# simonamtoft/downsampled-diffusion

Measured on AMD Instinct MI355X. Metric: images/sec (T=1000 sampling), 256x256 dDDPM-x3, higher is better.
Workload: dtype f32

## Files before the change

downsampled-diffusion_amd/csrc/level_chain.h:

```cpp
#pragma once
#include "ddk_internal.h"

namespace ddk {

constexpr int CH_MAX_OPS = 24;
enum ChainKind {
    CH_CONV3 = 0,
    CH_CONV1 = 1,
    CH_ATTN = 2,
    CH_UPT = 3
};
enum ChainFlag {
    CHF_WAIT = 1,
    CHF_SIGNAL = 2,
    CHF_ADD_KEEP = 4,
    CHF_SAVE_KEEP = 8,
    CHF_ADD_KEEP2 = 16,
    CHF_SAVE_KEEP2 = 32,
    CHF_KEEP_FROM_SRC = 64,
    CHF_NO_OUT = 128,
    CHF_NO_GN = 256,
    CHF_DOWN = 512
};

struct ChainOp {
    const float* src0;
    const float* src1;
    const float* w;
    const float* bias;
    const float* gamma;
    const float* beta;
    float* out;
    int c0, c1, kind, flags, temb_off, n_out;
};

struct ChainParams {
    ChainOp op[CH_MAX_OPS];
    const float* temb;
    const long long* temb_rows;
    unsigned* cnt;
    unsigned* done;
    unsigned* fail;
    int n_ops, B, temb_stride;
    float gn_eps, ln_eps;
    int hw;
};

bool level_chain_device_ok();
size_t level_chain_lds_bytes();
int level_chain_launch(const ChainParams& p, hipStream_t st);
int level_chain_init_device();

}
```

downsampled-diffusion_amd/csrc/level_chain.hip:

```cpp
#include "level_chain.h"
#include "cluster_sync.h"
#include "conv_common.h"

#include <atomic>
#include <cstdlib>
#include <type_traits>
#include <utility>

namespace ddk {

typedef float f32x4 __attribute__((ext_vector_type(4)));

constexpr int LC_BIG = 18432;
constexpr int LC_PP = 36;
constexpr int LC_QP = 100;
constexpr int LC_RED = LC_BIG;
constexpr int LC_TILE = LC_RED + 64;
constexpr int LC_KS = LC_TILE + 576;
constexpr int LC_VS = LC_KS + 512;
constexpr int LC_QS = LC_VS + 512;
constexpr int LC_CS = LC_QS + 528;
constexpr int LC_SMAX = LC_CS + 1152;
constexpr int LC_ROWSTAT = LC_SMAX + 32;
constexpr int LC_CFOLD = LC_ROWSTAT + 32;
constexpr int LC_MISC = LC_CFOLD + 192;
constexpr int LC_PF = LC_MISC + 4;
constexpr int LC_FLOATS = LC_PF + 256;

size_t level_chain_lds_bytes() { return 100 * 1024; }
static_assert(LC_FLOATS * 4 <= 100 * 1024, "LDS carve-up");

__device__ __forceinline__ void ld_sc1_x1(f32x4& a, const float* pa) {
    asm volatile("global_load_dwordx4 %0, %1, off sc1\n\ts_waitcnt vmcnt(0)" : "=&v"(a) : "v"(pa) : "memory");
}
__device__ __forceinline__ void ld_sc1_x2(f32x4& a, f32x4& b, const float* pa, const float* pb) {
    asm volatile("global_load_dwordx4 %0, %2, off sc1\n\tglobal_load_dwordx4 %1, %3, off sc1\n\ts_waitcnt vmcnt(0)"
                 : "=&v"(a), "=&v"(b) : "v"(pa), "v"(pb) : "memory");
}
__device__ __forceinline__ void ld_sc1_x4(f32x4& a, f32x4& b, f32x4& c, f32x4& d, const float* pa, const float* pb, const float* pc, const float* pd) {
    asm volatile("global_load_dwordx4 %0, %4, off sc1\n\tglobal_load_dwordx4 %1, %5, off sc1\n\tglobal_load_dwordx4 %2, %6, off sc1\n\t"
                 "global_load_dwordx4 %3, %7, off sc1\n\ts_waitcnt vmcnt(0)"
                 : "=&v"(a), "=&v"(b), "=&v"(c), "=&v"(d) : "v"(pa), "v"(pb), "v"(pc), "v"(pd) : "memory");
}
__device__ __forceinline__ void st_sc1(float* p, f32x4 v) { asm volatile("global_store_dwordx4 %0, %1, off sc1\n\ts_nop 1" :: "v"(p), "v"(v) : "memory"); }

#ifdef DDK_TUNING
__device__ unsigned long long g_lc_stamps[9 * CH_MAX_OPS * 8];
#define LC_STAMP(c, k, i)                                                                                                   \
    do {                                                                                                                    \
        if ((c).tid == 0 && (c).watch >= 0) g_lc_stamps[((c).watch * CH_MAX_OPS + (k)) * 8 + (i)] = __builtin_amdgcn_s_memrealtime(); \
    } while (0)
#else
#define LC_STAMP(c, k, i) do { } while (0)
// ... 10 lines not shown
    const int b = __builtin_bit_cast(int, v);
    const float r0 = __builtin_bit_cast(float, __builtin_amdgcn_readlane(b, 0)), r1 = __builtin_bit_cast(float, __builtin_amdgcn_readlane(b, 16));
    const float r2 = __builtin_bit_cast(float, __builtin_amdgcn_readlane(b, 32)), r3 = __builtin_bit_cast(float, __builtin_amdgcn_readlane(b, 48));
    return (r0 + r1) + (r2 + r3);
}

template <int... I, class F>
__device__ __forceinline__ void static_for_lc_impl(std::integer_sequence<int, I...>, F&& f) { (f(std::integral_constant<int, I>{}), ...); }
template <int N, class F>
__device__ __forceinline__ void static_for_lc(F&& f) { static_for_lc_impl(std::make_integer_sequence<int, N>{}, f); }

struct ChainCtx {
    float* lds;
    int tid, lane, wave, b, nt;
    unsigned signals;
    float keep, keep2;
    float* misc;
    unsigned pf_dst;
    int nwaves, units3;
    int slot, slots;
    int watch, k;
};

__device__ __forceinline__ void chain_wait(const ChainParams& p, ChainCtx& c) {
    int* dead = reinterpret_cast<int*>(c.misc);
    if (c.tid == 0 && !*dead && cl_wait_ge<1>(p.cnt + c.b * 32, 8u * c.signals, p.fail)) *dead = 1;
    __syncthreads();
}

__device__ __forceinline__ void chain_prefetch(const ChainOp& o, const ChainCtx& c) {
    const int cin = o.c0 + o.c1;
    const float* base;
    int lines;
    if (o.kind == CH_ATTN) {
        if (c.nt >= 4) return;
        base = o.w + (size_t)c.nt * (cin >> 5) * 3072;
        lines = (cin >> 5) * 3072 / 32;
    } else {
        const int taps = o.kind == CH_CONV3 ? c.units3 : o.kind == CH_UPT ? 16 : 1;
        base = o.w + (size_t)c.nt * taps * (cin >> 5) * 1024;
        lines = taps * (cin >> 5) * 1024 / 32;
    }
    const int share = (lines + c.slots - 1) / c.slots;
    const int first = c.slot * share;
    const int n = lines - first < share ? lines - first : share;
    for (int i = c.wave * 64; i < n; i += c.nwaves * 64) {
        int line = first + i + c.lane;
        line = line < first + n ? line : first + n - 1;
        lds_dma16(base + (size_t)line * 32, c.pf_dst);
    }
}

__device__ __forceinline__ void chain_finish(const ChainParams& p, const ChainOp& o, ChainCtx& c, float y, int n0) {
    if (o.flags & CHF_ADD_KEEP) y += c.keep;
    if (o.flags & CHF_ADD_KEEP2) y += c.keep2;
    if (o.flags & CHF_SAVE_KEEP) c.keep = y;
    if (o.flags & CHF_SAVE_KEEP2) c.keep2 = y;
    if (!(o.flags & CHF_NO_OUT)) {
        const int yb = __builtin_bit_cast(int, y);
        const float y0 = __builtin_bit_cast(float, __builtin_amdgcn_update_dpp(0, yb, 0x00, 0xF, 0xF, true));
        const float y1 = __builtin_bit_cast(float, __builtin_amdgcn_update_dpp(0, yb, 0x55, 0xF, 0xF, true));
        const float y2 = __builtin_bit_cast(float, __builtin_amdgcn_update_dpp(0, yb, 0xAA, 0xF, 0xF, true));
        const float y3 = __builtin_bit_cast(float, __builtin_amdgcn_update_dpp(0, yb, 0xFF, 0xF, 0xF, true));
        if ((c.lane & 3) == 0) {
            float* dst = o.out + ((long long)c.b * 16 + (c.tid >> 5)) * o.n_out + n0 + (c.tid & 31);
            const f32x4 v{y0, y1, y2, y3};
            if (o.flags & CHF_SIGNAL) st_sc1(dst, v);
            else *reinterpret_cast<f32x4*>(dst) = v;
        }
    }
    if (o.flags & CHF_SIGNAL) {
        asm volatile("s_waitcnt vmcnt(0)" ::: "memory");
        if (c.lane == 0) {
            unsigned* lcnt = reinterpret_cast<unsigned*>(c.misc) + 1;
            if ((atomicAdd(lcnt, 1u) & 7u) == 7u) __hip_atomic_fetch_add(p.cnt + c.b * 32, 1u, __ATOMIC_RELAXED, __HIP_MEMORY_SCOPE_AGENT);
        }
    }
}

__device__ __forceinline__ void chain_stage(const ChainOp& o, ChainCtx& c, int cin, int pitch) {
    const int q4 = cin >> 2;
    auto addr = [&](int idx) -> const float* {
        const int row = idx / q4, ch = (idx - row * q4) << 2;
        const long long r = (long long)c.b * 16 + row;
        return ch < o.c0 ? o.src0 + r * o.c0 + ch : o.src1 + r * o.c1 + (ch - o.c0);
    };
    auto put = [&](int idx, f32x4 v) {
        const int row = idx / q4, ch = (idx - row * q4) << 2;
        *reinterpret_cast<f32x4*>(c.lds + row * pitch + ch) = v;
    };
    if (cin == 512) {
        f32x4 v0, v1, v2, v3;
        ld_sc1_x4(v0, v1, v2, v3, addr(c.tid), addr(c.tid + 512), addr(c.tid + 1024), addr(c.tid + 1536));
        put(c.tid, v0); put(c.tid + 512, v1); put(c.tid + 1024, v2); put(c.tid + 1536, v3);
    } else if (cin == 256) {
        f32x4 v0, v1;
        ld_sc1_x2(v0, v1, addr(c.tid), addr(c.tid + 512));
        put(c.tid, v0); put(c.tid + 512, v1);
    } else {
        f32x4 v0;
        ld_sc1_x1(v0, addr(c.tid));
        put(c.tid, v0);
    }
    if (c.tid < q4) *reinterpret_cast<f32x4*>(c.lds + 16 * pitch + (c.tid << 2)) = f32x4{0.f, 0.f, 0.f, 0.f};
}

__device__ __forceinline__ void chain_stage64(const ChainOp& o, ChainCtx& c) {
    const float* src = o.src0 + (long long)c.b * 64 * 256;
#pragma unroll
    for (int r0 = 0; r0 < 4096; r0 += 2048) {
        f32x4 v0, v1, v2, v3;
        ld_sc1_x4(v0, v1, v2, v3, src + (size_t)(r0 + c.tid) * 4, src + (size_t)(r0 + c.tid + 512) * 4, src + (size_t)(r0 + c.tid + 1024) * 4,
                  src + (size_t)(r0 + c.tid + 1536) * 4);
        auto put = [&](int idx, f32x4 v) { *reinterpret_cast<f32x4*>(c.lds + (idx >> 6) * 260 + ((idx & 63) << 2)) = v; };
        put(r0 + c.tid, v0); put(r0 + c.tid + 512, v1); put(r0 + c.tid + 1024, v2); put(r0 + c.tid + 1536, v3);
    }
    if (c.tid < 64) *reinterpret_cast<f32x4*>(c.lds + 64 * 260 + (c.tid << 2)) = f32x4{0.f, 0.f, 0.f, 0.f};
}

template <int NU>
__device__ __forceinline__ void chain_conv(const ChainParams& p, const ChainOp& o, ChainCtx& c) {
    float* lds = c.lds;
    const int tid = c.tid, lane = c.lane, wave = c.wave;
    const int m = lane & 15, kq = lane >> 4;
    const int n0 = c.nt << 5;
    const int cin = o.c0 + o.c1, pitch = cin + 4, nch = cin >> 5;
    const int taps = o.kind == CH_CONV3 ? 9 : 1;

    const float* wl = o.w + (size_t)c.nt * taps * nch * 1024 + lane * 4;
    float4 bA[2][2], bB[2][2], bC[2][2];
    int ltap = 0, lchunk = wave;
    auto norm = [&](int& tap, int& chunk) {
        while (chunk >= nch) { chunk -= nch; ++tap; }
    };
    norm(ltap, lchunk);
    auto load_b = [&](float4 (&bq)[2][2]) {
        const int unit = ltap < taps ? ltap * nch + lchunk : taps * nch - 1;
        const float* wp = wl + (size_t)unit * 1024;
        bq[0][0] = *reinterpret_cast<const float4*>(wp);
        bq[0][1] = *reinterpret_cast<const float4*>(wp + 256);
        bq[1][0] = *reinterpret_cast<const float4*>(wp + 512);
        bq[1][1] = *reinterpret_cast<const float4*>(wp + 768);
        lchunk += 8;
        norm(ltap, lchunk);
    };
    load_b(bA);
    load_b(bB);
    load_b(bC);
    const int col = tid & 31, row = tid >> 5;
    const int ch = n0 + col;
    float ga = 1.f, be = 0.f, sh = 0.f;
    if (o.kind == CH_CONV3 && !(o.flags & CHF_NO_GN)) { ga = o.gamma[ch]; be = o.beta[ch]; }
    if (o.temb_off >= 0) {
        const long long tr = p.temb_rows ? p.temb_rows[c.b] : c.b;
        sh = p.temb[tr * p.temb_stride + o.temb_off + ch];
    }
    const float cb = o.bias ? o.bias[ch] : 0.f;
    if (o.flags & CHF_KEEP_FROM_SRC) c.keep = o.src0[((long long)c.b * 16 + row) * o.c0 + ch];
    if (c.k + 1 < p.n_ops) chain_prefetch(p.op[c.k + 1], c);
    const bool down = NU == 1 && (o.flags & CHF_DOWN);

    LC_STAMP(c, c.k, 0);
    if (o.flags & CHF_WAIT) chain_wait(p, c);
    else __syncthreads();
    LC_STAMP(c, c.k, 1);
    if (down) chain_stage64(o, c);
    else chain_stage(o, c, cin, pitch);
    __syncthreads();
    LC_STAMP(c, c.k, 2);

    f32x4 acc[2];
    acc[0] = acc[1] = f32x4{0.f, 0.f, 0.f, 0.f};
    const int py = m >> 2, px = m & 3;
    if constexpr (NU > 0) {
        int a_tap[9];
#pragma unroll
        for (int t = 0; t < 9; ++t) {
            if (down) {
                const int yy = 2 * py + t / 3 - 1, xx = 2 * px + t % 3 - 1;
                const bool ok = (unsigned)yy < 8u && (unsigned)xx < 8u;
                a_tap[t] = (ok ? yy * 8 + xx : 64) * pitch + kq * 8 + (wave << 5);
            } else {
                const int yy = py + t / 3 - 1, xx = px + t % 3 - 1;
                const bool ok = (unsigned)yy < 4u && (unsigned)xx < 4u;
                a_tap[t] = (ok ? yy * 4 + xx : 16) * pitch + kq * 8 + (wave << 5);
            }
        }
        auto compute_at = [&](int t, int sub, const float4 (&bq)[2][2]) {
            const float* ap = lds + a_tap[t] + sub * 256;
            const float4 a0 = *reinterpret_cast<const float4*>(ap), a1 = *reinterpret_cast<const float4*>(ap + 4);
            const float av[8] = {a0.x, a0.y, a0.z, a0.w, a1.x, a1.y, a1.z, a1.w};
#pragma unroll
// ... 24 lines not shown
            const float* ap = lds + srow * pitch + (cchunk << 5) + kq * 8;
            const float4 a0 = *reinterpret_cast<const float4*>(ap), a1 = *reinterpret_cast<const float4*>(ap + 4);
            const float av[8] = {a0.x, a0.y, a0.z, a0.w, a1.x, a1.y, a1.z, a1.w};
#pragma unroll
            for (int kk = 0; kk < 8; ++kk) {
                acc[0] = __builtin_amdgcn_mfma_f32_16x16x4f32(av[kk], reinterpret_cast<const float*>(&bq[0][0])[kk], acc[0], 0, 0, 0);
                acc[1] = __builtin_amdgcn_mfma_f32_16x16x4f32(av[kk], reinterpret_cast<const float*>(&bq[1][0])[kk], acc[1], 0, 0, 0);
            }
            cchunk += 8;
            norm(ctap, cchunk);
        };
        while (ctap < taps) {
            compute(bA);
            load_b(bA);
            if (ctap < taps) compute(bB);
            load_b(bB);
            if (ctap < taps) compute(bC);
            load_b(bC);
        }
    }

    LC_STAMP(c, c.k, 3);
    __syncthreads();
#pragma unroll
    for (int nb = 0; nb < 2; ++nb)
#pragma unroll
        for (int r = 0; r < 4; ++r) lds[(wave * 16 + kq * 4 + r) * LC_PP + nb * 16 + m] = acc[nb][r];
    __syncthreads();
    float v = lds[row * LC_PP + col];
#pragma unroll
    for (int w = 1; w < 8; ++w) v += lds[(w * 16 + row) * LC_PP + col];
    v += cb;
    float y = v;
    if (o.kind == CH_CONV3 && !(o.flags & CHF_NO_GN)) {
        float* red = lds + LC_RED;
        const float mw = wave_sum_dpp(v) * (1.0f / 64.0f);
        const float dw = v - mw;
        const float m2w = wave_sum_dpp(dw * dw);
        if (lane == 0) { red[2 * wave] = mw; red[2 * wave + 1] = m2w; }
        __syncthreads();
        float msum = red[0], m2 = red[1];
#pragma unroll
        for (int w = 1; w < 8; ++w) { msum += red[2 * w]; m2 += red[2 * w + 1]; }
        const float mean = msum * 0.125f;
        float dev = 0.f;
#pragma unroll
        for (int w = 0; w < 8; ++w) { const float dm = red[2 * w] - mean; dev += dm * dm; }
        const float var = (m2 + 64.0f * dev) * (1.0f / 512.0f);
        const float rstd = 1.0f / sqrtf(var + p.gn_eps);
        y = mish_f((v - mean) * rstd * ga + be) + sh;
    }
    chain_finish(p, o, c, y, n0);
    if (o.flags & CHF_SIGNAL) ++c.signals;
    LC_STAMP(c, c.k, 4);
// ... 2 lines not shown
__device__ __forceinline__ void chain_upt(const ChainParams& p, const ChainOp& o, ChainCtx& c) {
    float* lds = c.lds;
    const int tid = c.tid, lane = c.lane, wave = c.wave;
    const int m = lane & 15, kq = lane >> 4;
    const int n0 = c.nt << 5;
    const int cin = o.c0, pitch = cin + 4, nch = cin >> 5;
    const float* wl = o.w + ((size_t)c.nt * 16 * nch + wave) * 1024 + lane * 4;
    float4 bA[2][2], bB[2][2], bC[2][2];
    int lu = 0;
    auto load_b = [&](float4 (&bq)[2][2]) {
        const float* wp = wl + (size_t)(lu < 16 ? lu : 15) * nch * 1024;
        bq[0][0] = *reinterpret_cast<const float4*>(wp);
        bq[0][1] = *reinterpret_cast<const float4*>(wp + 256);
        bq[1][0] = *reinterpret_cast<const float4*>(wp + 512);
        bq[1][1] = *reinterpret_cast<const float4*>(wp + 768);
        ++lu;
    };
    load_b(bA);
    load_b(bB);
    load_b(bC);
    const int col = tid & 31, row = tid >> 5;
    const float cb = o.bias ? o.bias[n0 + col] : 0.f;
    if (c.k + 1 < p.n_ops) chain_prefetch(p.op[c.k + 1], c);
    LC_STAMP(c, c.k, 0);
    if (o.flags & CHF_WAIT) chain_wait(p, c);
    else __syncthreads();
    LC_STAMP(c, c.k, 1);
    chain_stage(o, c, cin, pitch);
    __syncthreads();
    LC_STAMP(c, c.k, 2);
    f32x4 acc[4][2];
#pragma unroll
    for (int ph = 0; ph < 4; ++ph) acc[ph][0] = acc[ph][1] = f32x4{0.f, 0.f, 0.f, 0.f};
    const int y = m >> 2, x = m & 3;
    auto unit = [&](auto phc, auto tpc, const float4 (&bq)[2][2]) {
        constexpr int ph = decltype(phc)::value, tp = decltype(tpc)::value;
        constexpr int pyy = ph >> 1, pxx = ph & 1, ty = tp >> 1, tx = tp & 1;
        constexpr int dy = pyy == 0 ? (ty == 0 ? 0 : -1) : (ty == 0 ? 1 : 0);
        constexpr int dx = pxx == 0 ? (tx == 0 ? 0 : -1) : (tx == 0 ? 1 : 0);
        const int yy = y + dy, xx = x + dx;
        const bool ok = (unsigned)yy < 4u && (unsigned)xx < 4u;
        const float* ap = lds + (ok ? yy * 4 + xx : 16) * pitch + (wave << 5) + kq * 8;
        const float4 a0 = *reinterpret_cast<const float4*>(ap), a1 = *reinterpret_cast<const float4*>(ap + 4);
        const float av[8] = {a0.x, a0.y, a0.z, a0.w, a1.x, a1.y, a1.z, a1.w};
#pragma unroll
        for (int kk = 0; kk < 8; ++kk) {
            acc[ph][0] = __builtin_amdgcn_mfma_f32_16x16x4f32(av[kk], reinterpret_cast<const float*>(&bq[0][0])[kk], acc[ph][0], 0, 0, 0);
            acc[ph][1] = __builtin_amdgcn_mfma_f32_16x16x4f32(av[kk], reinterpret_cast<const float*>(&bq[1][0])[kk], acc[ph][1], 0, 0, 0);
        }
    };
    static_for_lc<16>([&](auto uc) {
        constexpr int u = decltype(uc)::value;
        using PH = std::integral_constant<int, u / 4>;
        using TP = std::integral_constant<int, u % 4>;
        if constexpr (u % 3 == 0) { unit(PH{}, TP{}, bA); load_b(bA); }
        else if constexpr (u % 3 == 1) { unit(PH{}, TP{}, bB); load_b(bB); }
        else { unit(PH{}, TP{}, bC); load_b(bC); }
    });
    LC_STAMP(c, c.k, 3);
    __syncthreads();
#pragma unroll
    for (int ph = 0; ph < 4; ++ph)
#pragma unroll
        for (int nb = 0; nb < 2; ++nb)
#pragma unroll
            for (int r = 0; r < 4; ++r) lds[((wave * 4 + ph) * 16 + kq * 4 + r) * LC_PP + nb * 16 + m] = acc[ph][nb][r];
    __syncthreads();
    float yv[4];
#pragma unroll
    for (int ph = 0; ph < 4; ++ph) {
        float s = lds[(ph * 16 + row) * LC_PP + col];
#pragma unroll
        for (int w = 1; w < 8; ++w) s += lds[((w * 4 + ph) * 16 + row) * LC_PP + col];
        yv[ph] = s + cb;
    }
    {
        float g[4][4];
#pragma unroll
        for (int k = 0; k < 4; ++k) {
            const int yb = __builtin_bit_cast(int, yv[k]);
            g[k][0] = __builtin_bit_cast(float, __builtin_amdgcn_update_dpp(0, yb, 0x00, 0xF, 0xF, true));
            g[k][1] = __builtin_bit_cast(float, __builtin_amdgcn_update_dpp(0, yb, 0x55, 0xF, 0xF, true));
            g[k][2] = __builtin_bit_cast(float, __builtin_amdgcn_update_dpp(0, yb, 0xAA, 0xF, 0xF, true));
            g[k][3] = __builtin_bit_cast(float, __builtin_amdgcn_update_dpp(0, yb, 0xFF, 0xF, 0xF, true));
        }
        const int j = lane & 3;
        f32x4 v;
#pragma unroll
        for (int q = 0; q < 4; ++q) v[q] = j == 0 ? g[0][q] : j == 1 ? g[1][q] : j == 2 ? g[2][q] : g[3][q];
        const int oy = 2 * (row >> 2) + (j >> 1), ox = 2 * (row & 3) + (j & 1);
        float* dst = o.out + ((long long)c.b * 64 + oy * 8 + ox) * o.n_out + n0 + (col & ~3);
        if (o.flags & CHF_SIGNAL) st_sc1(dst, v);
        else *reinterpret_cast<f32x4*>(dst) = v;
    }
    if (o.flags & CHF_SIGNAL) {
        asm volatile("s_waitcnt vmcnt(0)" ::: "memory");
        if (lane == 0) {
            unsigned* lcnt = reinterpret_cast<unsigned*>(c.misc) + 1;
            if ((atomicAdd(lcnt, 1u) & 7u) == 7u) __hip_atomic_fetch_add(p.cnt + c.b * 32, 1u, __ATOMIC_RELAXED, __HIP_MEMORY_SCOPE_AGENT);
        }
        ++c.signals;
    }
    LC_STAMP(c, c.k, 4);
}

__device__ __forceinline__ void chain_attn(const ChainParams& p, const ChainOp& o, ChainCtx& c) {
    float* lds = c.lds;
    const int tid = c.tid, lane = c.lane, wave = c.wave;
    if (c.k + 1 < p.n_ops) chain_prefetch(p.op[c.k + 1], c);
    if (c.k + 2 < p.n_ops) chain_prefetch(p.op[c.k + 2], c);
    if (c.nt < 4) {
        const int h = c.nt;
        const int m = lane & 15, kq = lane >> 4;
        const int C = o.c0, pitch = C + 4, nch = C >> 5;
        float* xs = lds;
        float* ks = lds + LC_KS;
        float* vs = lds + LC_VS;
        float* qs = lds + LC_QS;
        float* cs = lds + LC_CS;
        float* smax = lds + LC_SMAX;
        float* rowstat = lds + LC_ROWSTAT;
        float* cfold = lds + LC_CFOLD;
        const float* wl = o.w + (size_t)h * nch * 3072 + lane * 4;
        float4 bq[6][2];
        {
            const int chunk = wave < nch ? wave : nch - 1;
            const float* wp = wl + (size_t)chunk * 3072;
#pragma unroll
            for (int nb = 0; nb < 6; ++nb) {
                bq[nb][0] = *reinterpret_cast<const float4*>(wp + nb * 512);
                bq[nb][1] = *reinterpret_cast<const float4*>(wp + nb * 512 + 256);
            }
        }
        if (tid < 192) {
            const int n = tid % 96;
            const int colw = (n >> 5) * 128 + h * 32 + (n & 31);
            cfold[tid] = tid < 96 ? o.gamma[colw] : o.beta[colw];
        }
        LC_STAMP(c, c.k, 0);
        if (o.flags & CHF_WAIT) chain_wait(p, c);
        else __syncthreads();
        LC_STAMP(c, c.k, 1);
        chain_stage(o, c, C, pitch);
        __syncthreads();
        LC_STAMP(c, c.k, 2);
        {
            const int row = tid >> 5, sub = tid & 31;
            float s1 = 0.f;
            for (int ch = sub * 4; ch < C; ch += 128) {
                const float4 v = *reinterpret_cast<const float4*>(xs + row * pitch + ch);
                s1 += (v.x + v.y) + (v.z + v.w);
            }
#pragma unroll
            for (int of = 1; of < 32; of <<= 1) s1 += __shfl_xor(s1, of, 64);
            const float inv_c = 1.0f / (float)C;
            const float mean = s1 * inv_c;
            float s2 = 0.f;
            for (int ch = sub * 4; ch < C; ch += 128) {
                const float4 v = *reinterpret_cast<const float4*>(xs + row * pitch + ch);
                const float a0 = v.x - mean, a1 = v.y - mean, a2 = v.z - mean, a3 = v.w - mean;
                s2 += (a0 * a0 + a1 * a1) + (a2 * a2 + a3 * a3);
            }
#pragma unroll
            for (int of = 1; of < 32; of <<= 1) s2 += __shfl_xor(s2, of, 64);
            if (sub == 0) {
                const float r = 1.0f / (sqrtf(s2 * inv_c) + p.ln_eps);
                rowstat[2 * row] = r;
                rowstat[2 * row + 1] = r * mean;
// ... 2 lines not shown
        f32x4 acc[6];
#pragma unroll
        for (int nb = 0; nb < 6; ++nb) acc[nb] = f32x4{0.f, 0.f, 0.f, 0.f};
        for (int chunk = wave; chunk < nch; chunk += 8) {
            const float* ap = xs + m * pitch + (chunk << 5) + kq * 8;
            const float4 a0 = *reinterpret_cast<const float4*>(ap), a1 = *reinterpret_cast<const float4*>(ap + 4);
            const float av[8] = {a0.x, a0.y, a0.z, a0.w, a1.x, a1.y, a1.z, a1.w};
#pragma unroll
            for (int kk = 0; kk < 8; ++kk)
#pragma unroll
                for (int nb = 0; nb < 6; ++nb)
                    acc[nb] = __builtin_amdgcn_mfma_f32_16x16x4f32(av[kk], reinterpret_cast<const float*>(&bq[nb][0])[kk], acc[nb], 0, 0, 0);
            if (chunk + 8 < nch) {
                const float* wp = wl + (size_t)(chunk + 8) * 3072;
#pragma unroll
                for (int nb = 0; nb < 6; ++nb) {
                    bq[nb][0] = *reinterpret_cast<const float4*>(wp + nb * 512);
                    bq[nb][1] = *reinterpret_cast<const float4*>(wp + nb * 512 + 256);
                }
            }
        }
        LC_STAMP(c, c.k, 3);
        __syncthreads();
#pragma unroll
        for (int nb = 0; nb < 6; ++nb)
#pragma unroll
            for (int r = 0; r < 4; ++r) xs[(wave * 16 + kq * 4 + r) * LC_QP + nb * 16 + m] = acc[nb][r];
        __syncthreads();
        for (int e = tid; e < 16 * 96; e += 512) {
            const int row = e / 96, n = e - row * 96;
            float s = xs[row * LC_QP + n];
#pragma unroll
            for (int w = 1; w < 8; ++w) s += xs[(w * 16 + row) * LC_QP + n];
            const float v = rowstat[2 * row] * s - rowstat[2 * row + 1] * cfold[n] + cfold[96 + n];
            const int sel = n >> 5, d = n & 31;
            if (sel == 0) qs[row * 33 + d] = v;
            else if (sel == 1) ks[row * 32 + d] = v;
            else vs[row * 32 + d] = v;
        }
        __syncthreads();
        if (tid < 32) {
            float mx = ks[tid];
#pragma unroll
            for (int n = 1; n < 16; ++n) mx = fmaxf(mx, ks[n * 32 + tid]);
            smax[tid] = mx;
        }
        __syncthreads();
        ks[tid] = __expf(ks[tid] - smax[tid & 31]);
        __syncthreads();
        {
            const int d = tid >> 4, e0 = (tid & 15) << 1;
            float a0 = 0.f, a1 = 0.f, den = 0.f;
#pragma unroll
            for (int n = 0; n < 16; ++n) {
                const float kd = ks[n * 32 + d];
                a0 += kd * vs[n * 32 + e0];
                a1 += kd * vs[n * 32 + e0 + 1];
                den += kd;
            }
            const float inv = 1.0f / den;
            cs[d * 36 + e0] = a0 * inv;
            cs[d * 36 + e0 + 1] = a1 * inv;
        }
        __syncthreads();
        const int n = tid >> 5, e = tid & 31;
        float y = 0.f;
#pragma unroll
        for (int d = 0; d < 32; ++d) y += qs[n * 33 + d] * cs[d * 36 + e];
        chain_finish(p, o, c, y, h * 32);
    } else {
        if (o.flags & CHF_WAIT) chain_wait(p, c);
        if ((o.flags & CHF_SIGNAL) && tid == 0) __hip_atomic_fetch_add(p.cnt + c.b * 32, 1u, __ATOMIC_RELAXED, __HIP_MEMORY_SCOPE_AGENT);
    }
    if (o.flags & CHF_SIGNAL) ++c.signals;
    LC_STAMP(c, c.k, 4);
}

__global__ __launch_bounds__(512) void level_chain_kernel(const ChainParams p) {
    extern __shared__ __align__(16) float lds[];
    ChainCtx c;
    c.lds = lds;
    c.tid = threadIdx.x;
    c.lane = c.tid & 63;
    c.wave = __builtin_amdgcn_readfirstlane(c.tid >> 6);
    c.nt = blockIdx.x & 7;
    c.misc = lds + LC_MISC;
    c.pf_dst = (unsigned)(size_t)(__attribute__((address_space(3))) float*)(lds + LC_PF);
    c.nwaves = 8;
    c.units3 = 9;
    c.watch = blockIdx.x == 0 ? 0 : blockIdx.x == 100 ? 1 : blockIdx.x == 255 ? 2 : -1;
    c.k = 0;
    if (c.tid == 0) { *reinterpret_cast<int*>(lds + LC_MISC) = 0; reinterpret_cast<unsigned*>(lds + LC_MISC)[1] = 0u; }
    __syncthreads();
    const int slots = gridDim.x >> 3;
    c.slot = blockIdx.x >> 3;
    c.slots = slots;
    for (int b = blockIdx.x >> 3; b < p.B; b += slots) {
        c.b = b;
        c.signals = 0;
        c.keep = c.keep2 = 0.f;
        chain_prefetch(p.op[0], c);
        for (int k = 0; k < p.n_ops; ++k) {
            const ChainOp& o = p.op[k];
            c.k = k;
            if (o.kind == CH_ATTN) chain_attn(p, o, c);
            else if (o.kind == CH_UPT) chain_upt(p, o, c);
            else if (o.kind == CH_CONV1) chain_conv<0>(p, o, c);
            else if (o.c0 + o.c1 == 256) chain_conv<1>(p, o, c);
            else if (o.c0 + o.c1 == 512) chain_conv<2>(p, o, c);
            else chain_conv<0>(p, o, c);
        }
        __syncthreads();
        if (c.tid == 0) cl_depart(p.cnt + b * 32, p.done + b * 32, 8u);
    }
}

constexpr int L8_P = 260;
constexpr int L8_IMG = 65 * L8_P;
constexpr int L8_VP = 36;
constexpr int L8_VBUF = 16 * 16 * L8_VP;
constexpr int L8_V = L8_IMG;
constexpr int L8_KS = L8_V;
constexpr int L8_VS = L8_KS + 2048;
constexpr int L8_QS = L8_VS + 2048;
constexpr int L8_CS = L8_QS + 2112;
constexpr int L8_RED = L8_V + 2 * L8_VBUF;
constexpr int L8_SMAX = L8_RED + 64;
constexpr int L8_ROWSTAT = L8_SMAX + 320;
constexpr int L8_CFOLD = L8_ROWSTAT + 128;
constexpr int L8_MISC = L8_CFOLD + 192;
constexpr int L8_PF = L8_MISC + 4;
constexpr int L8_FLOATS = L8_PF + 256;
static_assert(L8_CS + 1152 <= L8_RED, "attention arrays fit the V buffers");
static_assert(L8_FLOATS * 4 <= 160 * 1024, "LDS carve-up (8x8)");
static_assert(2 * 64 * LC_QP <= L8_IMG && 8 * 64 * LC_PP <= 2 * L8_VBUF, "partial tiles fit");

// ... 82 lines not shown
        }
    };
    const int tt = (tid >> 5) & 15, col = tid & 31, ch = n0 + col;
    const int tty = tt >> 2, ttx = tt & 3;
    float ga = 1.f, be = 0.f, sh = 0.f, cb = 0.f;
    if (matrix) {
        load_b(0, bA);
        load_b(1, bB);
        ga = o.gamma[ch]; be = o.beta[ch];
        if (o.temb_off >= 0) {
            const long long tr = p.temb_rows ? p.temb_rows[c.b] : c.b;
            sh = p.temb[tr * p.temb_stride + o.temb_off + ch];
        }
        if (o.bias) cb = o.bias[ch];
        if (o.flags & CHF_KEEP_FROM_SRC) {
#pragma unroll
            for (int k = 0; k < 4; ++k)
                kp.keep[k] = o.src0[((long long)c.b * 64 + (2 * tty + (k >> 1)) * 8 + 2 * ttx + (k & 1)) * o.c0 + ch];
        }
    }
    if (c.k + 1 < p.n_ops) chain_prefetch(p.op[c.k + 1], c);

    LC_STAMP(c, c.k, 0);
    if (o.flags & CHF_WAIT) chain_wait(p, c);
    else __syncthreads();
    LC_STAMP(c, c.k, 1);

    f32x4 acc[2][2];
    acc[0][0] = acc[0][1] = acc[1][0] = acc[1][1] = f32x4{0.f, 0.f, 0.f, 0.f};
    if (!matrix) {
        const int t2 = tid - 512;
        const int ftt = (t2 >> 5) & 15, ri = (t2 >> 3) & 3, q4i = t2 & 7;
        const int fty = ftt >> 2, ftx = ftt & 3;
        const int row_a = ri == 0 ? 0 : ri == 2 ? 2 : 1, row_b = ri == 0 ? 2 : ri == 1 ? 2 : ri == 2 ? 1 : 3;
        int poff[8];
#pragma unroll
        for (int hh = 0; hh < 2; ++hh)
#pragma unroll
            for (int j = 0; j < 4; ++j) {
                const int yy = 2 * fty - 1 + (hh == 0 ? row_a : row_b), xx = 2 * ftx - 1 + j;
                const bool ok = (unsigned)yy < 8u && (unsigned)xx < 8u;
                poff[hh * 4 + j] = (ok ? yy * 8 + xx : 64) * L8_P + q4i * 4;
            }
        const int voff = (4 * ri * 16 + ftt) * L8_VP + q4i * 4;
        const float sgn = ri == 1 ? 1.0f : -1.0f;
        auto f4 = [](const float* q) { return *reinterpret_cast<const float4*>(q); };
        auto sub4 = [](float4 a, float4 b) { return make_float4(a.x - b.x, a.y - b.y, a.z - b.z, a.w - b.w); };
// ... 104 lines not shown
        const float rstd = 1.0f / sqrtf(var + p.gn_eps);
#pragma unroll
        for (int k = 0; k < 4; ++k) v[k] = mish_f((v[k] - mean) * rstd * ga + be) + sh;
        c8_finish(p, o, c, kp, v, n0);
    }
    if (o.flags & CHF_SIGNAL) ++c.signals;
    LC_STAMP(c, c.k, 4);
}

__device__ __forceinline__ void c8_conv1(const ChainParams& p, const ChainOp& o, ChainCtx& c, C8Keep& kp) {
    float* lds = c.lds;
    const int tid = c.tid, lane = c.lane, wave = c.wave;
    const int m = lane & 15, kq = lane >> 4;
    const int n0 = c.nt << 5;
    const int cin = o.c0 + o.c1, nch = cin >> 5, halves = cin > 256 ? 2 : 1, hcols = cin > 256 ? 256 : cin, hch = hcols >> 5;
    const bool matrix = wave < 8;
    float* V = lds + L8_V;
    const float* wl = o.w + (size_t)c.nt * nch * 1024 + lane * 4;
    const int tt = (tid >> 5) & 15, col = tid & 31, ch = n0 + col;
    float cb = 0.f;
    if (matrix && o.bias) cb = o.bias[ch];
    if (c.k + 1 < p.n_ops) chain_prefetch(p.op[c.k + 1], c);
    LC_STAMP(c, c.k, 0);
    if (o.flags & CHF_WAIT) chain_wait(p, c);
    else __syncthreads();
    LC_STAMP(c, c.k, 1);
    f32x4 acc[4][2];
#pragma unroll
    for (int i = 0; i < 4; ++i) acc[i][0] = acc[i][1] = f32x4{0.f, 0.f, 0.f, 0.f};
    for (int hf = 0; hf < halves; ++hf) {
        if (hf > 0) __syncthreads();
        c8_stage(o, c, hf << 8, hcols);
        __syncthreads();
        if (hf == 0) LC_STAMP(c, c.k, 2);
        if (matrix) {
            const int pitch = hcols + 4;
            for (int lc = wave; lc < hch; lc += 8) {
                const float* wp = wl + (size_t)(hf * 8 + lc) * 1024;
                const float4 b00 = *reinterpret_cast<const float4*>(wp), b01 = *reinterpret_cast<const float4*>(wp + 256);
                const float4 b10 = *reinterpret_cast<const float4*>(wp + 512), b11 = *reinterpret_cast<const float4*>(wp + 768);
                const float bv0[8] = {b00.x, b00.y, b00.z, b00.w, b01.x, b01.y, b01.z, b01.w};
                const float bv1[8] = {b10.x, b10.y, b10.z, b10.w, b11.x, b11.y, b11.z, b11.w};
#pragma unroll
                for (int i = 0; i < 4; ++i) {
                    const float* ap = lds + (i * 16 + m) * pitch + (lc << 5) + kq * 8;
                    const float4 a0 = *reinterpret_cast<const float4*>(ap), a1 = *reinterpret_cast<const float4*>(ap + 4);
                    const float av[8] = {a0.x, a0.y, a0.z, a0.w, a1.x, a1.y, a1.z, a1.w};
// ... 38 lines not shown
    const int tid = c.tid, lane = c.lane, wave = c.wave;
    if (c.k + 1 < p.n_ops) chain_prefetch(p.op[c.k + 1], c);
    if (c.k + 2 < p.n_ops) chain_prefetch(p.op[c.k + 2], c);
    if (c.nt < 4) {
        const int h = c.nt;
        const int m = lane & 15, kq = lane >> 4;
        const int C = o.c0, nch = C >> 5;
        const bool matrix = wave < 8;
        float* xs = lds;
        float* ks = lds + L8_KS;
        float* vs = lds + L8_VS;
        float* qs = lds + L8_QS;
        float* cs = lds + L8_CS;
        float* smax = lds + L8_SMAX;
        float* rowstat = lds + L8_ROWSTAT;
        float* cfold = lds + L8_CFOLD;
        const float* wl = o.w + (size_t)h * nch * 3072 + lane * 4;
        if (tid < 192) {
            const int n = tid % 96;
            const int colw = (n >> 5) * 128 + h * 32 + (n & 31);
            cfold[tid] = tid < 96 ? o.gamma[colw] : o.beta[colw];
        }
        LC_STAMP(c, c.k, 0);
        if (o.flags & CHF_WAIT) chain_wait(p, c);
        else __syncthreads();
        LC_STAMP(c, c.k, 1);
        c8_stage(o, c, 0, C);
        __syncthreads();
        LC_STAMP(c, c.k, 2);
        {
            const int row = tid >> 4, sub = tid & 15;
            float s1 = 0.f;
            for (int chn = sub * 4; chn < C; chn += 64) {
                const float4 v = *reinterpret_cast<const float4*>(xs + row * L8_P + chn);
                s1 += (v.x + v.y) + (v.z + v.w);
            }
#pragma unroll
            for (int of = 1; of < 16; of <<= 1) s1 += __shfl_xor(s1, of, 64);
            const float inv_c = 1.0f / (float)C;
            const float mean = s1 * inv_c;
            float s2 = 0.f;
            for (int chn = sub * 4; chn < C; chn += 64) {
                const float4 v = *reinterpret_cast<const float4*>(xs + row * L8_P + chn);
                const float a0 = v.x - mean, a1 = v.y - mean, a2 = v.z - mean, a3 = v.w - mean;
                s2 += (a0 * a0 + a1 * a1) + (a2 * a2 + a3 * a3);
            }
#pragma unroll
// ... 69 lines not shown
                const float kd = ks[n * 32 + d];
                a += kd * vs[n * 32 + e];
                den += kd;
            }
            cs[d * 36 + e] = a * (1.0f / den);
        }
        __syncthreads();
        if (matrix) {
            const int tt = (tid >> 5) & 15, e = tid & 31;
            const int tty = tt >> 2, ttx = tt & 3;
            float y[4] = {0.f, 0.f, 0.f, 0.f};
            const int r00 = (2 * tty) * 8 + 2 * ttx;
#pragma unroll 4
            for (int d = 0; d < 32; ++d) {
                const float cv = cs[d * 36 + e];
                y[0] += qs[r00 * 33 + d] * cv;
                y[1] += qs[(r00 + 1) * 33 + d] * cv;
                y[2] += qs[(r00 + 8) * 33 + d] * cv;
                y[3] += qs[(r00 + 9) * 33 + d] * cv;
            }
            c8_finish(p, o, c, kp, y, h * 32);
        }
    } else {
        if (o.flags & CHF_WAIT) chain_wait(p, c);
        if ((o.flags & CHF_SIGNAL) && tid == 0) __hip_atomic_fetch_add(p.cnt + c.b * 32, 1u, __ATOMIC_RELAXED, __HIP_MEMORY_SCOPE_AGENT);
    }
    if (o.flags & CHF_SIGNAL) ++c.signals;
    LC_STAMP(c, c.k, 4);
}

__global__ __launch_bounds__(1024) void level8_chain_kernel(const ChainParams p) {
    extern __shared__ __align__(16) float lds[];
    ChainCtx c;
    c.lds = lds;
    c.tid = threadIdx.x;
    c.lane = c.tid & 63;
    c.wave = __builtin_amdgcn_readfirstlane(c.tid >> 6);
    c.nt = blockIdx.x & 7;
    c.misc = lds + L8_MISC;
    c.pf_dst = (unsigned)(size_t)(__attribute__((address_space(3))) float*)(lds + L8_PF);
    c.nwaves = 16;
    c.units3 = 16;
    c.watch = blockIdx.x == 0 ? 0 : blockIdx.x == 100 ? 1 : blockIdx.x == 255 ? 2 : -1;
    if (c.watch >= 0) c.watch += p.n_ops == 6 ? 3 : 6;
    c.k = 0;
    c.keep = c.keep2 = 0.f;
    if (c.tid == 0) { *reinterpret_cast<int*>(c.misc) = 0; reinterpret_cast<unsigned*>(c.misc)[1] = 0u; }
// ... 27 lines not shown
unsigned level_chain_cluster_timeouts() { return cl_timeouts_read(); }

int level_chain_init_device() {
    DDK_HIP(hipFuncSetAttribute(reinterpret_cast<const void*>(level_chain_kernel), hipFuncAttributeMaxDynamicSharedMemorySize, 160 * 1024));
    DDK_HIP(hipFuncSetAttribute(reinterpret_cast<const void*>(level8_chain_kernel), hipFuncAttributeMaxDynamicSharedMemorySize, 160 * 1024));
    return DDK_OK;
}

int level_chain_launch(const ChainParams& p, hipStream_t st) {
    DDK_REQUIRE(p.n_ops > 0 && p.n_ops <= CH_MAX_OPS && p.B > 0 && p.cnt && p.done && p.fail && (p.hw == 16 || p.hw == 64), "level_chain: arguments");
    for (int k = 0; k < p.n_ops; ++k) {
        const ChainOp& o = p.op[k];
        const int cin = o.c0 + o.c1;
        DDK_REQUIRE(o.src0 && o.w && aligned16(o.src0) && aligned16(o.src1) && aligned16(o.w) && aligned16(o.out), "level_chain: op pointers");
        DDK_REQUIRE((cin == 128 || cin == 256 || cin == 512) && o.c0 % 4 == 0 && o.c1 % 4 == 0 && (o.c1 == 0 || o.src1), "level_chain: op channels");
        if (p.hw == 64) {
            DDK_REQUIRE(o.kind != CH_CONV3 || cin == 256 || (cin == 512 && o.c0 == 256), "level_chain: 8x8 conv3x3 takes 256 channels, or 256 + 256");
            DDK_REQUIRE(o.kind != CH_CONV1 || cin == 128 || cin == 256 || (cin == 512 && o.c0 == 256), "level_chain: 8x8 conv1x1 channels");
            DDK_REQUIRE(o.kind != CH_ATTN || cin == 256, "level_chain: 8x8 attention takes 256 channels");
        }
        DDK_REQUIRE((o.flags & CHF_NO_OUT) || o.out, "level_chain: op output");
        if (o.kind == CH_ATTN) DDK_REQUIRE(o.c1 == 0 && o.n_out == 128 && o.gamma && o.beta, "level_chain: attention op");
        else DDK_REQUIRE(o.n_out == 256 && (o.kind != CH_CONV3 || (o.flags & CHF_NO_GN) || (o.gamma && o.beta)), "level_chain: conv op (8 slices of 32 channels)");
        if (o.flags & CHF_DOWN) DDK_REQUIRE(p.hw == 16 && o.kind == CH_CONV3 && cin == 256 && o.c1 == 0, "level_chain: stride-2 conv (4x4 chain, 256 channels)");
        if (o.kind == CH_UPT) DDK_REQUIRE(p.hw == 16 && cin == 256 && o.c1 == 0, "level_chain: transpose conv (4x4 chain, 256 channels)");
    }
    DDK_TRY(ensure_device_init());
    const int slots = p.B < 32 ? p.B : 32;
    if (p.hw == 64) {
        hipLaunchKernelGGL(level8_chain_kernel, dim3(8 * slots), dim3(1024), (size_t)L8_FLOATS * 4, st, p);
        return check_launch("level8_chain_kernel");
    }
    hipLaunchKernelGGL(level_chain_kernel, dim3(8 * slots), dim3(512), level_chain_lds_bytes(), st, p);
    return check_launch("level_chain_kernel");
}

}

extern "C" int ddk_debug_level_chain(const void* ops, int n, int hw, int B, const float* temb, int temb_stride, void* counters, ddk_stream_t s) {
    using namespace ddk;
    DDK_REQUIRE(ops && n > 0 && n <= CH_MAX_OPS && counters, "debug_level_chain: arguments");
    if (!level_chain_device_ok()) return fail_arg("debug_level_chain: needs a whole MI355X");
    ChainParams p{};
    const ChainOp* src = static_cast<const ChainOp*>(ops);
    for (int i = 0; i < n; ++i) p.op[i] = src[i];
    p.n_ops = n;
    p.B = B;
    p.hw = hw;
    p.temb = temb;
    p.temb_rows = nullptr;
    p.temb_stride = temb_stride;
    p.cnt = static_cast<unsigned*>(counters);
    p.done = p.cnt + (size_t)B * 32;
    p.fail = p.cnt + (size_t)B * 64;
    p.gn_eps = 1e-5f;
    p.ln_eps = 1e-5f;
    return level_chain_launch(p, as_stream(s));
}

#ifdef DDK_TUNING
extern "C" int ddk_debug_read_lc_stamps(unsigned long long* host_out) {
    if (hipDeviceSynchronize() != hipSuccess) return -2;
    return hipMemcpyFromSymbol(host_out, HIP_SYMBOL(ddk::g_lc_stamps), sizeof(unsigned long long) * 9 * ddk::CH_MAX_OPS * 8) == hipSuccess ? 0 : -2;
}
#endif
```

Measured before the change: 26.02.

## Replace whole-image chain barrier with per-slice counters and per-wave band staging

In the 4x4 level chain, each of the 8 blocks per image now publishes to its own counter word, and every wave waits only on the slice of channels it stages. Each wave loads its own 32-channel band instead of the whole block waiting on one aggregated counter and then staging cooperatively. Partial-sum reduction moves to a dedicated LDS region so staging and reduction no longer alias, and the LDS allocation grows to fit. This aims to let blocks start work as soon as their inputs are ready rather than waiting for all producers. The cost is more counter traffic, a larger LDS footprint that may reduce occupancy, and a new debug-only skew path for testing ordering.

Measured after the change: 26.17 (median of 6 runs). About the same (+0.6%).

```diff
diff --git a/downsampled-diffusion_amd/csrc/level_chain.h b/downsampled-diffusion_amd/csrc/level_chain.h
--- a/downsampled-diffusion_amd/csrc/level_chain.h
+++ b/downsampled-diffusion_amd/csrc/level_chain.h
@@ -44,6 +44,7 @@
     int n_ops, B, temb_stride;
     float gn_eps, ln_eps;
     int hw;
+    unsigned skew;
 };
 
 bool level_chain_device_ok();
diff --git a/downsampled-diffusion_amd/csrc/level_chain.hip b/downsampled-diffusion_amd/csrc/level_chain.hip
--- a/downsampled-diffusion_amd/csrc/level_chain.hip
+++ b/downsampled-diffusion_amd/csrc/level_chain.hip
@@ -11,10 +11,11 @@
 
 typedef float f32x4 __attribute__((ext_vector_type(4)));
 
-constexpr int LC_BIG = 18432;
+constexpr int LC_IMG = 0;
+constexpr int LC_PART = LC_IMG + 65 * 260;
 constexpr int LC_PP = 36;
 constexpr int LC_QP = 100;
-constexpr int LC_RED = LC_BIG;
+constexpr int LC_RED = LC_PART + 8 * 64 * LC_PP;
 constexpr int LC_TILE = LC_RED + 64;
 constexpr int LC_KS = LC_TILE + 576;
 constexpr int LC_VS = LC_KS + 512;
@@ -27,8 +28,9 @@
 constexpr int LC_PF = LC_MISC + 4;
 constexpr int LC_FLOATS = LC_PF + 256;
 
-size_t level_chain_lds_bytes() { return 100 * 1024; }
-static_assert(LC_FLOATS * 4 <= 100 * 1024, "LDS carve-up");
+size_t level_chain_lds_bytes() { return (size_t)LC_FLOATS * 4; }
+static_assert(17 * 516 <= LC_PART - LC_IMG && 16 * 100 * 8 <= LC_RED - LC_PART && LC_PART % 4 == 0, "LDS regions");
+static_assert(LC_FLOATS * 4 <= 160 * 1024, "LDS carve-up");
 
 __device__ __forceinline__ void ld_sc1_x1(f32x4& a, const float* pa) {
     asm volatile("global_load_dwordx4 %0, %1, off sc1\n\ts_waitcnt vmcnt(0)" : "=&v"(a) : "v"(pa) : "memory");
@@ -85,7 +87,40 @@
     int watch, k;
 };
 
-__device__ __forceinline__ void chain_wait(const ChainParams& p, ChainCtx& c) {
+__device__ __forceinline__ unsigned* chain_word(const ChainParams& p, int b, int s) { return p.cnt + b * 32 + s * 4; }
+
+__device__ __forceinline__ void chain_wait_slice(const ChainParams& p, const ChainCtx& c, int s) {
+    int* dead = reinterpret_cast<int*>(c.misc);
+    if (c.lane == 0 && !*dead && cl_wait_ge<1>(chain_word(p, c.b, s), c.signals, p.fail)) *dead = 1;
+}
+
+__device__ __forceinline__ void chain_arrive(const ChainParams& p, const ChainCtx& c) {
+    if (p.skew) {
+        const unsigned long long t0 = __builtin_amdgcn_s_memrealtime();
+        const unsigned long long d = (unsigned long long)p.skew * (unsigned)((c.nt * 5 + c.k * 3 + c.b) & 7);
+        while (__builtin_amdgcn_s_memrealtime() - t0 < d) __builtin_amdgcn_s_sleep(2);
+    }
+    __hip_atomic_fetch_add(chain_word(p, c.b, c.nt), 1u, __ATOMIC_RELAXED, __HIP_MEMORY_SCOPE_AGENT);
+}
+
+__device__ __forceinline__ void chain_publish(const ChainParams& p, const ChainCtx& c) {
+    asm volatile("s_waitcnt vmcnt(0)" ::: "memory");
+    if (c.lane == 0) {
+        unsigned* lcnt = reinterpret_cast<unsigned*>(c.misc) + 1;
+        if ((atomicAdd(lcnt, 1u) & 7u) == 7u) chain_arrive(p, c);
+    }
+}
+
+__device__ __forceinline__ void chain_depart(const ChainParams& p, int b) {
+    unsigned* done = p.done + b * 32;
+    if (__hip_atomic_fetch_add(done, 1u, __ATOMIC_RELAXED, __HIP_MEMORY_SCOPE_AGENT) == 7u) {
+#pragma unroll
+        for (int s = 0; s < 8; ++s) __hip_atomic_store(chain_word(p, b, s), 0u, __ATOMIC_RELAXED, __HIP_MEMORY_SCOPE_AGENT);
+        __hip_atomic_store(done, 0u, __ATOMIC_RELAXED, __HIP_MEMORY_SCOPE_AGENT);
+    }
+}
+
+__device__ __forceinline__ void c8_wait(const ChainParams& p, ChainCtx& c) {
     int* dead = reinterpret_cast<int*>(c.misc);
     if (c.tid == 0 && !*dead && cl_wait_ge<1>(p.cnt + c.b * 32, 8u * c.signals, p.fail)) *dead = 1;
     __syncthreads();
@@ -132,53 +167,56 @@
             else *reinterpret_cast<f32x4*>(dst) = v;
         }
     }
-    if (o.flags & CHF_SIGNAL) {
-        asm volatile("s_waitcnt vmcnt(0)" ::: "memory");
-        if (c.lane == 0) {
-            unsigned* lcnt = reinterpret_cast<unsigned*>(c.misc) + 1;
-            if ((atomicAdd(lcnt, 1u) & 7u) == 7u) __hip_atomic_fetch_add(p.cnt + c.b * 32, 1u, __ATOMIC_RELAXED, __HIP_MEMORY_SCOPE_AGENT);
-        }
-    }
-}
-
-__device__ __forceinline__ void chain_stage(const ChainOp& o, ChainCtx& c, int cin, int pitch) {
-    const int q4 = cin >> 2;
-    auto addr = [&](int idx) -> const float* {
-        const int row = idx / q4, ch = (idx - row * q4) << 2;
-        const long long r = (long long)c.b * 16 + row;
-        return ch < o.c0 ? o.src0 + r * o.c0 + ch : o.src1 + r * o.c1 + (ch - o.c0);
+    if (o.flags & CHF_SIGNAL) chain_publish(p, c);
+}
+
+__device__ __forceinline__ void chain_stage_band(const ChainOp& o, const ChainCtx& c, int cin, int pitch) {
+    if ((c.wave << 5) >= cin) return;
+    const int r = c.lane >> 3, ch = (c.wave << 5) + ((c.lane & 7) << 2);
+    auto addr = [&](int row, int chn) -> const float* {
+        const long long rr = (long long)c.b * 16 + row;
+        return chn < o.c0 ? o.src0 + rr * o.c0 + chn : o.src1 + rr * o.c1 + (chn - o.c0);
     };
-    auto put = [&](int idx, f32x4 v) {
-        const int row = idx / q4, ch = (idx - row * q4) << 2;
-        *reinterpret_cast<f32x4*>(c.lds + row * pitch + ch) = v;
-    };
+    auto put = [&](int row, int chn, f32x4 v) { *reinterpret_cast<f32x4*>(c.lds + LC_IMG + row * pitch + chn) = v; };
+    const f32x4 zero{0.f, 0.f, 0.f, 0.f};
     if (cin == 512) {
         f32x4 v0, v1, v2, v3;
-        ld_sc1_x4(v0, v1, v2, v3, addr(c.tid), addr(c.tid + 512), addr(c.tid + 1024), addr(c.tid + 1536));
-        put(c.tid, v0); put(c.tid + 512, v1); put(c.tid + 1024, v2); put(c.tid + 1536, v3);
-    } else if (cin == 256) {
+        ld_sc1_x4(v0, v1, v2, v3, addr(r, ch), addr(r + 8, ch), addr(r, ch + 256), addr(r + 8, ch + 256));
+        put(r, ch, v0); put(r + 8, ch, v1); put(r, ch + 256, v2); put(r + 8, ch + 256, v3);
+        if (r == 0) { put(16, ch, zero); put(16, ch + 256, zero); }
+    } else {
         f32x4 v0, v1;
-        ld_sc1_x2(v0, v1, addr(c.tid), addr(c.tid + 512));
-        put(c.tid, v0); put(c.tid + 512, v1);
-    } else {
-        f32x4 v0;
-        ld_sc1_x1(v0, addr(c.tid));
-        put(c.tid, v0);
-    }
-    if (c.tid < q4) *reinterpret_cast<f32x4*>(c.lds + 16 * pitch + (c.tid << 2)) = f32x4{0.f, 0.f, 0.f, 0.f};
-}
-
-__device__ __forceinline__ void chain_stage64(const ChainOp& o, ChainCtx& c) {
-    const float* src = o.src0 + (long long)c.b * 64 * 256;
-#pragma unroll
-    for (int r0 = 0; r0 < 4096; r0 += 2048) {
+        ld_sc1_x2(v0, v1, addr(r, ch), addr(r + 8, ch));
+        put(r, ch, v0); put(r + 8, ch, v1);
+        if (r == 0) put(16, ch, zero);
+    }
+}
+
+__device__ __forceinline__ void chain_stage64_band(const ChainOp& o, const ChainCtx& c) {
+    const int r = c.lane >> 3, ch = (c.wave << 5) + ((c.lane & 7) << 2);
+    const float* src = o.src0 + ((long long)c.b * 64 + r) * 256 + ch;
+    float* dst = c.lds + LC_IMG + r * 260 + ch;
+#pragma unroll
+    for (int r0 = 0; r0 < 64; r0 += 32) {
         f32x4 v0, v1, v2, v3;
-        ld_sc1_x4(v0, v1, v2, v3, src + (size_t)(r0 + c.tid) * 4, src + (size_t)(r0 + c.tid + 512) * 4, src + (size_t)(r0 + c.tid + 1024) * 4,
-                  src + (size_t)(r0 + c.tid + 1536) * 4);
-        auto put = [&](int idx, f32x4 v) { *reinterpret_cast<f32x4*>(c.lds + (idx >> 6) * 260 + ((idx & 63) << 2)) = v; };
-        put(r0 + c.tid, v0); put(r0 + c.tid + 512, v1); put(r0 + c.tid + 1024, v2); put(r0 + c.tid + 1536, v3);
-    }
-    if (c.tid < 64) *reinterpret_cast<f32x4*>(c.lds + 64 * 260 + (c.tid << 2)) = f32x4{0.f, 0.f, 0.f, 0.f};
+        ld_sc1_x4(v0, v1, v2, v3, src + (r0 + 0) * 256, src + (r0 + 8) * 256, src + (r0 + 16) * 256, src + (r0 + 24) * 256);
+        *reinterpret_cast<f32x4*>(dst + (r0 + 0) * 260) = v0;
+        *reinterpret_cast<f32x4*>(dst + (r0 + 8) * 260) = v1;
+        *reinterpret_cast<f32x4*>(dst + (r0 + 16) * 260) = v2;
+        *reinterpret_cast<f32x4*>(dst + (r0 + 24) * 260) = v3;
+    }
+    if (r == 0) *reinterpret_cast<f32x4*>(c.lds + LC_IMG + 64 * 260 + ch) = f32x4{0.f, 0.f, 0.f, 0.f};
+}
+
+__device__ __forceinline__ void chain_front(const ChainParams& p, const ChainOp& o, const ChainCtx& c, int cin, int pitch, bool whole) {
+    LC_STAMP(c, c.k, 0);
+    if (o.flags & CHF_WAIT) chain_wait_slice(p, c, c.wave);
+    LC_STAMP(c, c.k, 1);
+    if (o.flags & CHF_DOWN) chain_stage64_band(o, c);
+    else chain_stage_band(o, c, cin, pitch);
+    if (whole) __syncthreads();
+    else asm volatile("s_waitcnt lgkmcnt(0)" ::: "memory");
+    LC_STAMP(c, c.k, 2);
 }
 
 template <int NU>
@@ -223,14 +261,7 @@
     if (c.k + 1 < p.n_ops) chain_prefetch(p.op[c.k + 1], c);
     const bool down = NU == 1 && (o.flags & CHF_DOWN);
 
-    LC_STAMP(c, c.k, 0);
-    if (o.flags & CHF_WAIT) chain_wait(p, c);
-    else __syncthreads();
-    LC_STAMP(c, c.k, 1);
-    if (down) chain_stage64(o, c);
-    else chain_stage(o, c, cin, pitch);
-    __syncthreads();
-    LC_STAMP(c, c.k, 2);
+    chain_front(p, o, c, cin, pitch, NU == 0 && taps == 9 && nch < 8);
 
     f32x4 acc[2];
     acc[0] = acc[1] = f32x4{0.f, 0.f, 0.f, 0.f};
@@ -301,14 +332,15 @@
 
     LC_STAMP(c, c.k, 3);
     __syncthreads();
+    float* part = lds + LC_PART;
 #pragma unroll
     for (int nb = 0; nb < 2; ++nb)
 #pragma unroll
-        for (int r = 0; r < 4; ++r) lds[(wave * 16 + kq * 4 + r) * LC_PP + nb * 16 + m] = acc[nb][r];
+        for (int r = 0; r < 4; ++r) part[(wave * 16 + kq * 4 + r) * LC_PP + nb * 16 + m] = acc[nb][r];
     __syncthreads();
-    float v = lds[row * LC_PP + col];
-#pragma unroll
-    for (int w = 1; w < 8; ++w) v += lds[(w * 16 + row) * LC_PP + col];
+    float v = part[row * LC_PP + col];
+#pragma unroll
+    for (int w = 1; w < 8; ++w) v += part[(w * 16 + row) * LC_PP + col];
     v += cb;
     float y = v;
     if (o.kind == CH_CONV3 && !(o.flags & CHF_NO_GN)) {
@@ -357,13 +389,7 @@
     const int col = tid & 31, row = tid >> 5;
     const float cb = o.bias ? o.bias[n0 + col] : 0.f;
     if (c.k + 1 < p.n_ops) chain_prefetch(p.op[c.k + 1], c);
-    LC_STAMP(c, c.k, 0);
-    if (o.flags & CHF_WAIT) chain_wait(p, c);
-    else __syncthreads();
-    LC_STAMP(c, c.k, 1);
-    chain_stage(o, c, cin, pitch);
-    __syncthreads();
-    LC_STAMP(c, c.k, 2);
+    chain_front(p, o, c, cin, pitch, false);
     f32x4 acc[4][2];
 #pragma unroll
     for (int ph = 0; ph < 4; ++ph) acc[ph][0] = acc[ph][1] = f32x4{0.f, 0.f, 0.f, 0.f};
@@ -394,19 +420,20 @@
     });
     LC_STAMP(c, c.k, 3);
     __syncthreads();
+    float* part = lds + LC_PART;
 #pragma unroll
     for (int ph = 0; ph < 4; ++ph)
 #pragma unroll
         for (int nb = 0; nb < 2; ++nb)
 #pragma unroll
-            for (int r = 0; r < 4; ++r) lds[((wave * 4 + ph) * 16 + kq * 4 + r) * LC_PP + nb * 16 + m] = acc[ph][nb][r];
+            for (int r = 0; r < 4; ++r) part[((wave * 4 + ph) * 16 + kq * 4 + r) * LC_PP + nb * 16 + m] = acc[ph][nb][r];
     __syncthreads();
     float yv[4];
 #pragma unroll
     for (int ph = 0; ph < 4; ++ph) {
-        float s = lds[(ph * 16 + row) * LC_PP + col];
-#pragma unroll
-        for (int w = 1; w < 8; ++w) s += lds[((w * 4 + ph) * 16 + row) * LC_PP + col];
+        float s = part[(ph * 16 + row) * LC_PP + col];
+#pragma unroll
+        for (int w = 1; w < 8; ++w) s += part[((w * 4 + ph) * 16 + row) * LC_PP + col];
         yv[ph] = s + cb;
     }
     {
@@ -429,11 +456,7 @@
         else *reinterpret_cast<f32x4*>(dst) = v;
     }
     if (o.flags & CHF_SIGNAL) {
-        asm volatile("s_waitcnt vmcnt(0)" ::: "memory");
-        if (lane == 0) {
-            unsigned* lcnt = reinterpret_cast<unsigned*>(c.misc) + 1;
-            if ((atomicAdd(lcnt, 1u) & 7u) == 7u) __hip_atomic_fetch_add(p.cnt + c.b * 32, 1u, __ATOMIC_RELAXED, __HIP_MEMORY_SCOPE_AGENT);
-        }
+        chain_publish(p, c);
         ++c.signals;
     }
     LC_STAMP(c, c.k, 4);
@@ -472,13 +495,7 @@
             const int colw = (n >> 5) * 128 + h * 32 + (n & 31);
             cfold[tid] = tid < 96 ? o.gamma[colw] : o.beta[colw];
         }
-        LC_STAMP(c, c.k, 0);
-        if (o.flags & CHF_WAIT) chain_wait(p, c);
-        else __syncthreads();
-        LC_STAMP(c, c.k, 1);
-        chain_stage(o, c, C, pitch);
-        __syncthreads();
-        LC_STAMP(c, c.k, 2);
+        chain_front(p, o, c, C, pitch, true);
         {
             const int row = tid >> 5, sub = tid & 31;
             float s1 = 0.f;
@@ -527,16 +544,17 @@
         }
         LC_STAMP(c, c.k, 3);
         __syncthreads();
+        float* part = lds + LC_PART;
 #pragma unroll
         for (int nb = 0; nb < 6; ++nb)
 #pragma unroll
-            for (int r = 0; r < 4; ++r) xs[(wave * 16 + kq * 4 + r) * LC_QP + nb * 16 + m] = acc[nb][r];
+            for (int r = 0; r < 4; ++r) part[(wave * 16 + kq * 4 + r) * LC_QP + nb * 16 + m] = acc[nb][r];
         __syncthreads();
         for (int e = tid; e < 16 * 96; e += 512) {
             const int row = e / 96, n = e - row * 96;
-            float s = xs[row * LC_QP + n];
-#pragma unroll
-            for (int w = 1; w < 8; ++w) s += xs[(w * 16 + row) * LC_QP + n];
+            float s = part[row * LC_QP + n];
+#pragma unroll
+            for (int w = 1; w < 8; ++w) s += part[(w * 16 + row) * LC_QP + n];
             const float v = rowstat[2 * row] * s - rowstat[2 * row + 1] * cfold[n] + cfold[96 + n];
             const int sel = n >> 5, d = n & 31;
             if (sel == 0) qs[row * 33 + d] = v;
@@ -574,8 +592,10 @@
         for (int d = 0; d < 32; ++d) y += qs[n * 33 + d] * cs[d * 36 + e];
         chain_finish(p, o, c, y, h * 32);
     } else {
-        if (o.flags & CHF_WAIT) chain_wait(p, c);
-        if ((o.flags & CHF_SIGNAL) && tid == 0) __hip_atomic_fetch_add(p.cnt + c.b * 32, 1u, __ATOMIC_RELAXED, __HIP_MEMORY_SCOPE_AGENT);
+        if (o.flags & CHF_SIGNAL) {
+            __syncthreads();
+            if (tid == 0) chain_arrive(p, c);
+        }
     }
     if (o.flags & CHF_SIGNAL) ++c.signals;
     LC_STAMP(c, c.k, 4);
@@ -616,7 +636,7 @@
             else chain_conv<0>(p, o, c);
         }
         __syncthreads();
-        if (c.tid == 0) cl_depart(p.cnt + b * 32, p.done + b * 32, 8u);
+        if (c.tid == 0) chain_depart(p, b);
     }
 }
 
@@ -745,7 +765,7 @@
     if (c.k + 1 < p.n_ops) chain_prefetch(p.op[c.k + 1], c);
 
     LC_STAMP(c, c.k, 0);
-    if (o.flags & CHF_WAIT) chain_wait(p, c);
+    if (o.flags & CHF_WAIT) c8_wait(p, c);
     else __syncthreads();
     LC_STAMP(c, c.k, 1);
 
@@ -896,7 +916,7 @@
     if (matrix && o.bias) cb = o.bias[ch];
     if (c.k + 1 < p.n_ops) chain_prefetch(p.op[c.k + 1], c);
     LC_STAMP(c, c.k, 0);
-    if (o.flags & CHF_WAIT) chain_wait(p, c);
+    if (o.flags & CHF_WAIT) c8_wait(p, c);
     else __syncthreads();
     LC_STAMP(c, c.k, 1);
     f32x4 acc[4][2];
@@ -981,7 +1001,7 @@
             cfold[tid] = tid < 96 ? o.gamma[colw] : o.beta[colw];
         }
         LC_STAMP(c, c.k, 0);
-        if (o.flags & CHF_WAIT) chain_wait(p, c);
+        if (o.flags & CHF_WAIT) c8_wait(p, c);
         else __syncthreads();
         LC_STAMP(c, c.k, 1);
         c8_stage(o, c, 0, C);
@@ -1097,7 +1117,7 @@
             c8_finish(p, o, c, kp, y, h * 32);
         }
     } else {
-        if (o.flags & CHF_WAIT) chain_wait(p, c);
+        if (o.flags & CHF_WAIT) c8_wait(p, c);
         if ((o.flags & CHF_SIGNAL) && tid == 0) __hip_atomic_fetch_add(p.cnt + c.b * 32, 1u, __ATOMIC_RELAXED, __HIP_MEMORY_SCOPE_AGENT);
     }
     if (o.flags & CHF_SIGNAL) ++c.signals;
@@ -1171,6 +1191,7 @@
         DDK_REQUIRE((o.flags & CHF_NO_OUT) || o.out, "level_chain: op output");
         if (o.kind == CH_ATTN) DDK_REQUIRE(o.c1 == 0 && o.n_out == 128 && o.gamma && o.beta, "level_chain: attention op");
         else DDK_REQUIRE(o.n_out == 256 && (o.kind != CH_CONV3 || (o.flags & CHF_NO_GN) || (o.gamma && o.beta)), "level_chain: conv op (8 slices of 32 channels)");
+        if (p.hw == 16) DDK_REQUIRE(o.c1 == 0 || o.c0 == 256, "level_chain: 4x4 concat takes 256 + c1 channels");
         if (o.flags & CHF_DOWN) DDK_REQUIRE(p.hw == 16 && o.kind == CH_CONV3 && cin == 256 && o.c1 == 0, "level_chain: stride-2 conv (4x4 chain, 256 channels)");
         if (o.kind == CH_UPT) DDK_REQUIRE(p.hw == 16 && cin == 256 && o.c1 == 0, "level_chain: transpose conv (4x4 chain, 256 channels)");
     }
@@ -1186,7 +1207,8 @@
 
 }
 
-extern "C" int ddk_debug_level_chain(const void* ops, int n, int hw, int B, const float* temb, int temb_stride, void* counters, ddk_stream_t s) {
+static int debug_level_chain(const void* ops, int n, int hw, int B, const float* temb, int temb_stride, void* counters, unsigned skew,
+                             ddk_stream_t s) {
     using namespace ddk;
     DDK_REQUIRE(ops && n > 0 && n <= CH_MAX_OPS && counters, "debug_level_chain: arguments");
     if (!level_chain_device_ok()) return fail_arg("debug_level_chain: needs a whole MI355X");
@@ -1204,7 +1226,19 @@
     p.fail = p.cnt + (size_t)B * 64;
     p.gn_eps = 1e-5f;
     p.ln_eps = 1e-5f;
+    p.skew = skew;
     return level_chain_launch(p, as_stream(s));
+}
+
+extern "C" int ddk_debug_level_chain(const void* ops, int n, int hw, int B, const float* temb, int temb_stride, void* counters, ddk_stream_t s) {
+    return debug_level_chain(ops, n, hw, B, temb, temb_stride, counters, 0u, s);
+}
+
+extern "C" int ddk_debug_level_chain_skewed(const void* ops, int n, int hw, int B, const float* temb, int temb_stride, void* counters,
+                                            unsigned skew_ticks, ddk_stream_t s) {
+    using namespace ddk;
+    DDK_REQUIRE(hw == 16 && skew_ticks < 1000u, "debug_level_chain_skewed: 4x4 chain, skew < 10 us");
+    return debug_level_chain(ops, n, hw, B, temb, temb_stride, counters, skew_ticks, s);
 }
 
 #ifdef DDK_TUNING
```
